# jdm365/Compression_Algorithms

Hardware: AMD Instinct MI355X
Metric: encode GB/s on enwik9 at 1/2/4/8 MI355X; ratio vs ref; round-trip bit-exact (higher is better)
Workload: dtype u8; 1 GPU; deflate (LZ77 W=32 KiB len<=31 + per-block dynamic Huffman over the 286-symbol alphabet, mode H), independent 64 KiB blocks; 1000000000 enwik-shaped bytes in the job, 1000000000 on rank 0; input_seed=12345, mode=H, input_bytes_job=1000000000, input_bytes_rank0=1000000000, compressed_bytes_job=516875560, compressed_bytes_rank0=516875560, gather_to_rank0=False, parallelism=blocks sharded over 1 GPU(s), weak scaling

## Files before the change

### compression_algorithms_amd/csrc/lz2.h

```cpp
#pragma once
#include "lz_common.h"

#define LZ2_NG_BITS   14
#define LZ2_NG        (1u << LZ2_NG_BITS)
#ifndef LZ2_CAP
#define LZ2_CAP       4096u
#endif
#ifndef LZ2_CAP_S
#define LZ2_CAP_S     2560u
#endif
#ifndef LZ2_THREADS
#define LZ2_THREADS   512
#endif
#define LZ2_NWAVES    (LZ2_THREADS / 64)
#ifndef LZ2_PARTBITS
#define LZ2_PARTBITS  7
#endif
#define LZ2_MAXPARTS  (1u << LZ2_PARTBITS)
static_assert(LZ2_CAP % LZ2_THREADS == 0 && LZ2_CAP_S % LZ2_THREADS == 0 && LZ2_CAP_S <= LZ2_CAP, "entries per thread must be whole");
static_assert(2u * (LZ_MAX_BLOCK / LZ2_CAP_S + 1u + 16u) + 2u <= LZ2_MAXPARTS, "a block could need more parts than the partition can number");
#define LZ2_GRID_PARTS 32u
#ifndef LZ2_BIG
#define LZ2_BIG       8u
#endif
#define LZ2_WAVE      128u
#define LZ2_MAXBIG    (LZ2_CAP / LZ2_BIG)
#define LZ2_BIG_STRIDE (2u * LZ_MAX_BLOCK)
#define LZ2_ALIGN8(x)  (((x) + 7u) & ~7u)
#define LZ2_DESC_SMALL (LZ_MAX_BLOCK / LZ2_BIG + 32u)
#define LZ2_NCLASS    8u
#define LZ2_BIG_SMALL 1024u
__host__ __device__ __forceinline__ uint32_t lz2_class_of(uint32_t cnt, uint32_t wave_min)
{
    const bool three = (wave_min >> 16) != 0u;
    wave_min &= 0xFFFFu;
    if (cnt >= wave_min) return cnt > LZ2_BIG_SMALL ? 6u : cnt >= 512u ? 4u : (three && cnt < 256u) ? 3u : 5u;
    return cnt < 16 ? 7u : cnt < 32 ? 0u : cnt < 64 ? 1u : cnt < 128 ? 2u : cnt < 256 ? 3u : 4u;
}

struct Lz2BlockMeta {
    uint32_t n, nparts, base, fallback;
    uint32_t nbig, nbig_entries;
    uint32_t pad[2];
    uint32_t part_start[LZ2_MAXPARTS];
    uint32_t part_count[LZ2_MAXPARTS];
    uint32_t part_lo[LZ2_MAXPARTS];
};

struct Lz2BigDesc {
    uint32_t block;
    uint32_t start;
    uint32_t count;
    uint32_t anom;
    uint32_t limit;
// ... 20 lines not shown
```

### compression_algorithms_amd/csrc/lz2_find.hip

```cpp
#include "lz_common.h"
#include "lz2.h"
#include "lz_dom.h"
#include "lz_replay.h"
#include <stdlib.h>

#define RS_HEAD 0x8000u
#define RS_MASK 0x7FFFu

__device__ __forceinline__ bool bm2_test(const uint32_t *bm, uint32_t b) { return (bm[b >> 5] >> (b & 31u)) & 1u; }

__device__ void replay_small(const uint16_t *pos, uint16_t *rs, const uint16_t *pid, uint16_t *occ, uint32_t *bm,
                             uint32_t s, uint32_t e, uint32_t W, uint32_t anom, uint32_t limit, uint16_t *cand_i)
{
    uint32_t ev = s;
    bool anom_pending = anom != ~0u;
    const bool plain = (anom == ~0u) && (limit == ~0u);
    if (plain && (uint32_t)pos[e - 1] <= (uint32_t)pos[s] + W) {
        for (uint32_t i = s; i < e; ++i) { const uint32_t id = pid[i]; cand_i[i] = (id != pos[i]) ? (uint16_t)id : (uint16_t)LZ_NONE16; }
        return;
    }
    for (uint32_t i = s; i < e; ++i) {
        const uint32_t p = pos[i], rsv = rs[i], r = rsv & RS_MASK, id = pid[i];
        while (ev < i && (uint32_t)pos[ev] + W < p) {
            const uint32_t b = rs[ev] & RS_MASK;
// ... 45 lines not shown
        const uint32_t i = s + li;
        const uint32_t p = pos[i], rr = ((uint32_t)rs[i] & RS_MASK) - s, id = pid[i];
        while (ev < li && ev_pos + W < p) {
            mask &= ~(1u << ((uint32_t)(slots >> (4u * ev)) & 15u));
            ++ev; ev_pos = pos[s + ev];
        }
        uint32_t res = LZ_NONE16;
        if (ev == 0) {
            if (id != p) res = id;
        } else if (id != p) {
            for (uint32_t b = rr; (mask >> b) & 1u; ++b) {
                const uint32_t o = s + ((uint32_t)(ent >> (4u * b)) & 15u);
                if (pid[o] == id) { res = pos[o]; break; }
            }
        }
        cand_i[i] = (uint16_t)res;
        const uint32_t b = rr + (uint32_t)__builtin_ctz(~(mask >> rr));
        mask |= 1u << b;
        ent = (ent & ~((F)15u << (4u * b))) | ((F)li << (4u * b));
        slots |= (F)b << (4u * li);
    }
}

template <uint32_t CAP>
__device__ __forceinline__ void lz2_find_part(const uint8_t *__restrict__ in, uint64_t n_total, const LzP &P, const Lz2Scratch &sc, uint64_t block0, const uint64_t item)
{
    __shared__ uint16_t s_pos[CAP];
    __shared__ uint32_t s_word[CAP];
    __shared__ uint16_t s_j0[CAP], s_j1[CAP];
    __shared__ __attribute__((aligned(16))) uint16_t s_gr[2 * CAP];
    uint16_t *const s_g = s_gr;
    uint16_t *const s_r = s_gr + CAP;
    __shared__ uint16_t s_pid[CAP + 2];
    __shared__ uint32_t s_cnt[LZ2_NWAVES + 1][256];
    __shared__ uint32_t s_bm[CAP / 32 + 2];
    __shared__ uint32_t s_mix[CAP / 32 + 2];
    __shared__ int32_t  s_i32[18];
    __shared__ uint32_t s_zslot, s_zgid, s_nbigl, s_ngroups;
    uint16_t *const s_gstart = s_pid;
    uint32_t *const s_big = &s_cnt[0][0];
    uint16_t *const s_quiet = reinterpret_cast<uint16_t *>(&s_cnt[0][0] + 3 * (CAP / LZ2_BIG));
    static_assert(3 * (CAP / LZ2_BIG) * 4 + 2 * (CAP / LZ2_BIG) * 2 <= sizeof(uint32_t) * LZ2_NWAVES * 256, "export lists must fit the radix counters");

    const int tid = threadIdx.x;
    const uint32_t lb = (uint32_t)item & 0xFFFFu, part = (uint32_t)(item >> 16) & 0xFFu;
    Lz2BlockMeta *mt = sc.meta + lb;
    long long tk = clock64();
#ifdef MI_MEASURE
#define LZ2_STOP(k) if ((k) < 7 && sc.stop_phase == (uint32_t)(k) + 1u) return
#else
#define LZ2_STOP(k) do { } while (0)
#endif
#define LZ2_TICK(k) do { if (sc.dbg && tid == 0) { long long t2 = clock64(); atomicAdd((unsigned long long *)&sc.dbg[k], (unsigned long long)(t2 - tk)); tk = t2; } \
                         LZ2_STOP(k); } while (0)
    const uint32_t m = (uint32_t)(item >> 24) & 0xFFFFu;
    if (m == 0) return;
    const uint32_t pstart = (uint32_t)(item >> 40), base = mt->base;
    const uint64_t off = (block0 + lb) * (uint64_t)P.block;
    const uint32_t nblk = mt->n;
    const uint8_t *src = in + off;
    const uint32_t T = 1u << P.tbits, Tmask = T - 1u, W = 1u << P.wbits;
    uint16_t *plist = sc.plist + (size_t)lb * LZ_MAX_BLOCK + pstart;
    (void)n_total;
    const uint32_t plo_ = mt->part_lo[part];
    const uint32_t phi_ = (part + 1 < mt->nparts) ? mt->part_lo[part + 1] : T;
    const bool three = (phi_ - plo_) > 65536u;
    uint32_t *const cntA = &s_cnt[0][0];
    uint32_t (*const s_cntB)[256] = reinterpret_cast<uint32_t (*)[256]>(s_gr);
    uint32_t *const cntB = &s_cntB[0][0];
    constexpr uint32_t RST = LZ2_NWAVES + 1;
    const uint32_t seg = radix_seg<LZ2_NWAVES>(m), seg_inv = (uint32_t)((0x100000000ull + seg - 1u) / seg);
    for (uint32_t i = tid; i < 256u * RST; i += LZ2_THREADS) { cntA[i] = 0; cntB[i] = 0; }

    bool viol = false;
    {
        constexpr uint32_t BPT = LZ_MAX_BLOCK / LZ2_THREADS;
        static_assert(BPT % 16u == 0, "whole 16-byte loads");
        const uint4 *pm = reinterpret_cast<const uint4 *>(sc.partmap + (size_t)lb * LZ_MAX_BLOCK + (size_t)tid * BPT);
        static_assert(BPT == 128u, "the match bitmap below is four dwords per thread");
        const uint32_t pat = part * 0x01010101u;
        auto nib = [&](uint32_t w) -> uint32_t {
            const uint32_t x = w ^ pat;
            const uint32_t z = ~(((x & 0x7F7F7F7Fu) + 0x7F7F7F7Fu) | x) & 0x80808080u;
            return (((z >> 7) * 0x00204081u) >> 21) & 15u;
        };
        uint32_t bm[4] = {0u, 0u, 0u, 0u};
        {
            uint4 pv[BPT / 16u];
#pragma unroll
            for (uint32_t q = 0; q < BPT / 16u; ++q) pv[q] = pm[q];
#pragma unroll
            for (uint32_t q = 0; q < BPT / 16u; ++q)
                bm[q >> 1] |= (nib(pv[q].x) | (nib(pv[q].y) << 4) | (nib(pv[q].z) << 8) | (nib(pv[q].w) << 12)) << (16u * (q & 1u));
        }
        const uint32_t mine = (uint32_t)(__popc(bm[0]) + __popc(bm[1]) + __popc(bm[2]) + __popc(bm[3]));
        __shared__ uint32_t s_scanp[LZ2_NWAVES + 2];
        uint32_t total_m;
        uint32_t at = block_exclusive_scan<uint32_t>(mine, OpAddU32(), 0u, s_scanp, &total_m);
        (void)total_m;
        const uint32_t p0 = (uint32_t)tid * BPT;
#pragma unroll
        for (uint32_t k = 0; k < 4; ++k) {
// ... 11 lines not shown
        constexpr uint32_t GCH = CAP / LZ2_THREADS;
        uint32_t gp[GCH], glo[GCH], ghi[GCH];
        const bool aligned = (((uintptr_t)src) & 3u) == 0;
#pragma unroll
        for (uint32_t c = 0; c < GCH; ++c) { const uint32_t j = tid + c * LZ2_THREADS; gp[c] = j < m ? (uint32_t)s_pos[j] : 0u; if (j < m) plist[j] = (uint16_t)gp[c]; }
#pragma unroll
        for (uint32_t c = 0; c < GCH; ++c) {
            const uint32_t j = tid + c * LZ2_THREADS, p = gp[c];
            glo[c] = 0; ghi[c] = 0;
            if (j < m) {
                if (p + 8 <= nblk && aligned) {
                    const uintptr_t a = (uintptr_t)(src + p) & ~(uintptr_t)3;
                    glo[c] = *reinterpret_cast<const uint32_t *>(a);
                    ghi[c] = *reinterpret_cast<const uint32_t *>(a + 4);
                } else {
                    uint32_t w = 0;
                    for (uint32_t k = 0; k < 4 && p + k < nblk; ++k) w |= (uint32_t)src[p + k] << (8 * k);
                    glo[c] = w;
                }
            }
        }
        __syncthreads();
#pragma unroll
        for (uint32_t c = 0; c < GCH; ++c) {
            const uint32_t j = tid + c * LZ2_THREADS, p = gp[c];
            if (j < m) {
                uint32_t w = glo[c];
                if (p + 8 <= nblk && aligned) {
                    const uint32_t sh = ((uint32_t)((uintptr_t)(src + p) & 3u)) * 8u;
                    if (sh) w = (glo[c] >> sh) | (ghi[c] << (32u - sh));
                }
                const uint32_t mx = lz_mix32(w);
                s_word[j] = mx;
                atomicAdd(&cntA[(((((mx & Tmask) - base) & Tmask) - plo_) & 255u) * RST + __umulhi(j, seg_inv)], 1u);
            }
        }
    }
    for (uint32_t i = tid; i < CAP / 32 + 2; i += LZ2_THREADS) { s_bm[i] = 0; s_mix[i] = 0; }
    if (tid == 0) { s_zslot = ~0u; s_zgid = ~0u; s_nbigl = 0; }
    __syncthreads();
    auto homep = [&](uint32_t j) -> uint32_t { return ((s_word[j] & Tmask) - base) & Tmask; };
    LZ2_TICK(0);

    const uint32_t arank = P.flags & (LZP_ARANK | LZP_BREAK);
    auto keyp = [&](uint32_t j) -> uint32_t { return homep(j) - plo_; };
    uint16_t *srt = s_j0;
    if (three) {
        radix_pass<LZ2_NWAVES, 8, uint32_t>(m, s_cnt, [&](uint32_t i) { return i; },
            [&](uint32_t e) { return keyp(e) & 255u; }, [&](uint32_t d, uint32_t e) { s_j0[d] = (uint16_t)e; }, arank, nullptr, true,
            [&](uint32_t d, uint32_t e) { atomicAdd(&cntB[((keyp(e) >> 8) & 255u) * RST + __umulhi(d, seg_inv)], 1u); });
        for (uint32_t i = tid; i < 256u * RST; i += LZ2_THREADS) cntA[i] = 0;
        radix_pass<LZ2_NWAVES, 8, uint32_t>(m, s_cntB, [&](uint32_t i) { return (uint32_t)s_j0[i]; },
            [&](uint32_t e) { return (keyp(e) >> 8) & 255u; }, [&](uint32_t d, uint32_t e) { s_j1[d] = (uint16_t)e; }, arank, nullptr, true,
            [&](uint32_t d, uint32_t e) { atomicAdd(&cntA[((keyp(e) >> 16) & 255u) * RST + __umulhi(d, seg_inv)], 1u); });
        radix_pass<LZ2_NWAVES, 8, uint32_t>(m, s_cnt, [&](uint32_t i) { return (uint32_t)s_j1[i]; },
            [&](uint32_t e) { return (keyp(e) >> 16) & 255u; }, [&](uint32_t d, uint32_t e) { s_j0[d] = (uint16_t)e; }, arank, nullptr, true);
    } else {
        radix_pass<LZ2_NWAVES, 8, uint32_t>(m, s_cnt, [&](uint32_t i) { return i; },
            [&](uint32_t e) { return keyp(e) & 255u; }, [&](uint32_t d, uint32_t e) { s_j1[d] = (uint16_t)e; }, arank, sc.dbg, true,
            [&](uint32_t d, uint32_t e) { atomicAdd(&cntB[((keyp(e) >> 8) & 255u) * RST + __umulhi(d, seg_inv)], 1u); });
        radix_pass<LZ2_NWAVES, 8, uint32_t>(m, s_cntB, [&](uint32_t i) { return (uint32_t)s_j1[i]; },
            [&](uint32_t e) { return (keyp(e) >> 8) & 255u; }, [&](uint32_t d, uint32_t e) { s_j0[d] = (uint16_t)e; }, arank, sc.dbg, true);
    }
    (void)srt;

    LZ2_TICK(1);
    constexpr uint32_t CH = CAP / LZ2_THREADS;
    const uint32_t k0 = tid * CH, k1 = (k0 + CH < m) ? k0 + CH : m;
    {
        uint32_t rj[CH], rw[CH]; int32_t rh[CH];
        int32_t mx = INT32_MIN;
#pragma unroll
        for (uint32_t c = 0; c < CH; ++c) {
            const uint32_t k = k0 + c;
            rj[c] = 0; rw[c] = 0; rh[c] = 0;
            if (k < k1) {
                rj[c] = s_j0[k]; rw[c] = s_word[rj[c]]; rh[c] = (int32_t)(((rw[c] & Tmask) - base) & Tmask);
                const int32_t g = rh[c] - (int32_t)k;
                mx = g > mx ? g : mx;
            }
        }
        int32_t gmax_total;
        const int32_t premax = block_exclusive_scan<int32_t>(mx, OpMaxI32(), INT32_MIN, s_i32, &gmax_total);
        int32_t prev_h0 = 0; uint32_t prev_j = 0;
        if (k0 > 0 && k0 < m) { prev_j = s_j0[k0 - 1]; prev_h0 = (int32_t)homep(prev_j); }
        uint32_t nheads = 0; int32_t lasthead = -1, lastrun = -1;
        {
            int32_t run = premax, prev_h = prev_h0;
#pragma unroll
            for (uint32_t c = 0; c < CH; ++c) {
                const uint32_t k = k0 + c;
                if (k < k1) {
                    const int32_t h = rh[c], g = h - (int32_t)k;
                    const bool head = (k == 0) || (g >= run);
                    run = g > run ? g : run;
// ... 57 lines not shown
                }
                s_pid[j] = s_pos[id];
            }
        }
    }
    if (viol) { lz_order_violation(P); viol = false; }
    __syncthreads();
    if (!P.deflate && W >= nblk) {
        uint16_t *cout = sc.cand + (size_t)lb * LZ_MAX_BLOCK + pstart;
        for (uint32_t j = tid; j < m; j += LZ2_THREADS) { const uint32_t id = s_pid[j]; cout[j] = (id != s_pos[j]) ? (uint16_t)id : (uint16_t)LZ_NONE16; }
        return;
    }
    if (tid == 0) {
        const uint32_t Z = (0u - base) & Tmask;
        const uint32_t plo = mt->part_lo[part];
        const uint32_t phi = (part + 1 < mt->nparts) ? mt->part_lo[part + 1] : T;
        if (Z >= plo && (Z < phi || phi == T)) {
            int32_t lo = -1, hi = (int32_t)m - 1;
            while (lo < hi) { const int32_t mid = (lo + hi + 1) >> 1; if (homep(s_j0[mid]) <= Z) lo = mid; else hi = mid - 1; }
            if (lo >= 0) {
                const uint32_t j = s_j0[lo], gid = s_g[j];
                const uint32_t slot = (uint32_t)s_r[j] + (Z - homep(j));
                int32_t a = lo, b = (int32_t)m - 1;
                while (a < b) { const int32_t mid = (a + b + 1) >> 1; if (s_g[s_j0[mid]] == gid) a = mid; else b = mid - 1; }
                if (slot <= (uint32_t)a) { s_zslot = slot; s_zgid = gid; }
            }
        }
    }
    __syncthreads();

    LZ2_TICK(2);
    static_assert(CAP <= 8192, "cluster numbers must fit 13 bits");
    constexpr int GB2 = CAP > 4096 ? 7 : 6;
    static_assert(2 * CAP <= sizeof(uint32_t) * (LZ2_NWAVES + 1) * 256, "the cluster cursors live in the radix counters");
    if (arank & LZP_ARANK) {
        uint32_t *cur32 = &s_cnt[0][0];
        const uint32_t wv = (uint32_t)tid >> 6, ln = (uint32_t)tid & 63u;
        auto multi = [&](uint32_t g) -> bool { return (s_bm[g >> 5] >> (g & 31u)) & 1u; };
        for (uint32_t k = k0; k < k1; ++k) { const uint32_t j = s_j0[k]; if (!multi(s_g[j])) s_j1[k] = (uint16_t)j; }
        __syncthreads();
        uint32_t nm;
        {
            uint32_t mine[CH], cnt = 0;
#pragma unroll
            for (uint32_t c = 0; c < CH; ++c) { const uint32_t j = k0 + c; mine[c] = (j < m && multi(s_g[j])) ? 1u : 0u; cnt += mine[c]; }
            uint32_t at = block_exclusive_scan<uint32_t>(cnt, OpAddU32(), 0u, reinterpret_cast<uint32_t *>(s_i32), &nm);
#pragma unroll
            for (uint32_t c = 0; c < CH; ++c) if (mine[c]) s_j0[at++] = (uint16_t)(k0 + c);
        }
        __syncthreads();
        for (uint32_t x0 = 0; x0 < nm; x0 += 256u) {
            uint32_t jj[4], gg[4], old[4];
#pragma unroll
            for (uint32_t u = 0; u < 4; ++u) { const uint32_t x = x0 + 64u * u + ln; jj[u] = x < nm ? (uint32_t)s_j0[x] : 0u; gg[u] = x < nm ? (uint32_t)s_g[jj[u]] : 0xFFFFFFFFu; }
#pragma unroll
            for (uint32_t u = 0; u < 4; ++u) {
                old[u] = 0;
                if (gg[u] != 0xFFFFFFFFu && ((gg[u] >> 1) % (uint32_t)LZ2_NWAVES) == wv) old[u] = atomicAdd(&cur32[gg[u] >> 1], 1u << (16u * (gg[u] & 1u)));
            }
#pragma unroll
            for (uint32_t u = 0; u < 4; ++u)
                if (gg[u] != 0xFFFFFFFFu && ((gg[u] >> 1) % (uint32_t)LZ2_NWAVES) == wv) s_j1[(old[u] >> (16u * (gg[u] & 1u))) & 0xFFFFu] = (uint16_t)jj[u];
        }
        __syncthreads();
        for (uint32_t i = tid; i < CAP / 32 + 2; i += LZ2_THREADS) s_bm[i] = 0;
    } else {
        radix_pass<LZ2_NWAVES, 6, uint32_t>(m, s_cnt, [&](uint32_t i) { return i; },
            [&](uint32_t e) { return (uint32_t)s_g[e] & 63u; }, [&](uint32_t d, uint32_t e) { s_j0[d] = (uint16_t)e; }, arank);
        radix_pass<LZ2_NWAVES, GB2, uint32_t>(m, s_cnt, [&](uint32_t i) { return (uint32_t)s_j0[i]; },
// ... 76 lines not shown
            for (int sz = (int)LZ2_BIG - 1; sz >= 2; --sz) { const uint32_t t = s_bin[sz]; s_bin[sz] = run; run += t; }
            s_ncl = run;
        }
        __syncthreads();
        for (uint32_t c = 0; c < CH; ++c)
            if (my_n[c] >= 2 && my_n[c] < LZ2_BIG) c_start[atomicAdd(&s_bin[my_n[c]], 1u)] = (uint16_t)my_s[c];
        __syncthreads();
        LZ2_TICK(12);
        nbig = s_nbigl < (CAP / LZ2_BIG) ? s_nbigl : (CAP / LZ2_BIG);
        {
            uint32_t it = 0;
            for (uint32_t q = tid; q < nbig; q += LZ2_THREADS, ++it) {
                const uint32_t cnt = s_big[3 * q + 1] - s_big[3 * q];
                const uint32_t cls = lz2_class_of(cnt, sc.wave_min);
                my_rank[it] = atomicAdd(&s_cls[cls], 1u);
                my_dst[it] = atomicAdd(&s_ent, LZ2_ALIGN8(cnt));
            }
        }
        __syncthreads();
        uint32_t pending_base = 0;
        const bool want_cls = tid < (int)LZ2_NCLASS && s_cls[tid], want_ent = tid == 32 && s_ent;
        if (want_cls || want_ent) {
            uint32_t *ap = want_ent ? &mt->nbig_entries : &sc.big_count[tid & (int)(LZ2_NCLASS - 1u)];
            pending_base = atomicAdd(ap, want_ent ? s_ent : s_cls[tid & (int)(LZ2_NCLASS - 1u)]);
        }
        if (want_ent) atomicAdd(&mt->nbig, nbig);
        for (uint32_t q = tid >> 6; q < s_nquiet; q += LZ2_NWAVES)
            for (uint32_t k = (uint32_t)s_quiet[2 * q] + (tid & 63u); k < s_quiet[2 * q + 1]; k += 64) {
                const uint32_t id = e_pid[k];
                cand_i[k] = (id != e_pos[k]) ? (uint16_t)id : (uint16_t)LZ_NONE16;
            }
        const uint32_t ncl = s_ncl;
        LZ2_TICK(13);
        if (sc.dbg && tid == 0) { atomicAdd((unsigned long long *)&sc.dbg[23], (unsigned long long)ncl); atomicAdd((unsigned long long *)&sc.dbg[24], (unsigned long long)nbig);
                                  atomicAdd((unsigned long long *)&sc.dbg[25], (unsigned long long)s_ent); atomicAdd((unsigned long long *)&sc.dbg[26], (unsigned long long)s_nquiet);
                                  atomicAdd((unsigned long long *)&sc.dbg[27], (unsigned long long)m); atomicAdd((unsigned long long *)&sc.dbg[28], (unsigned long long)s_ngroups); }
        for (uint32_t c = 0; c < CH; ++c) {
            const uint32_t i = tid + c * (uint32_t)LZ2_THREADS;
            if (i >= m) continue;
            const uint32_t g_ = regs[c][2] >> 16;
            if ((s_mix[g_ >> 5] >> (g_ & 31u)) & 1u) continue;
            const uint32_t s = s_gstart[g_];
            if (s == s_zhead || s_gstart[g_ + 1] - s < 2u) continue;
            const uint32_t p = regs[c][0];
            uint32_t a = e_pos[s], lo = s + 1u;
            while (a + W < p) {
                uint32_t hi = i;
                while (lo < hi) { const uint32_t mid = (lo + hi) >> 1; if ((uint32_t)e_pos[mid] > a + W) hi = mid; else lo = mid + 1u; }
                a = e_pos[lo]; ++lo;
            }
            cand_i[i] = (a == p) ? (uint16_t)LZ_NONE16 : (uint16_t)a;
        }
        for (uint32_t q = tid; q < ncl; q += LZ2_THREADS) {
            const uint32_t s = c_start[q];
            uint32_t e = s + 1;
            while (e < m && !(e_rs[e] & RS_HEAD)) ++e;
            const bool zc = (s == s_zhead);
            if (zc) replay_small(e_pos, e_rs, e_pid, occ, s_bm, s, e, W, s_zslot, P.deflate ? s_zslot : ~0u, cand_i);
            else if (LZ2_BIG > 8u && e - s >= 8u) replay_small_reg<uint64_t>(e_pos, e_rs, e_pid, s, e, W, cand_i);
            else replay_small_reg<uint32_t>(e_pos, e_rs, e_pid, s, e, W, cand_i);
        }
        if (want_cls) s_clsbase[tid] = pending_base;
        if (want_ent) s_entbase = pending_base;
    }
    __syncthreads();
    LZ2_TICK(5);
    {
        uint32_t it = 0;
        for (uint32_t q = tid; q < nbig; q += LZ2_THREADS, ++it) {
// ... 2 lines not shown
            const uint32_t dst = s_entbase + my_dst[it];
            s_big[3 * q + 2] = dst;
            Lz2BigDesc d;
            d.block = lb; d.start = dst; d.count = cnt;
            const bool zc = (s == s_zhead);
            d.anom = zc ? s_zslot - s : ~0u;
            d.limit = (zc && P.deflate) ? s_zslot - s : ~0u;
            d.pad[0] = pstart; d.pad[1] = d.pad[2] = 0;
            sc.desc[cls][s_clsbase[cls] + my_rank[it]] = d;
        }
    }
    __syncthreads();
    for (uint32_t b = tid >> 6; b < nbig; b += LZ2_NWAVES) {
        const uint32_t s = s_big[3 * b], e = s_big[3 * b + 1], dst = s_big[3 * b + 2];
        uint16_t *bp = sc.bigpos + (size_t)lb * LZ2_BIG_STRIDE + dst;
        uint16_t *br = sc.bigrs + (size_t)lb * LZ2_BIG_STRIDE + dst;
        uint16_t *bi = sc.bigpid + (size_t)lb * LZ2_BIG_STRIDE + dst;
        for (uint32_t i = s + (tid & 63); i < e; i += 64) {
            cand_i[i] = e_pos[i];
            bp[i - s] = e_pos[i];
            br[i - s] = (uint16_t)((e_rs[i] & RS_MASK) - s);
            bi[i - s] = e_pid[i];
        }
        uint16_t *bc = sc.bigcand + (size_t)lb * LZ2_BIG_STRIDE + dst;
        for (uint32_t k = (e - s) + (tid & 63); k < LZ2_ALIGN8(e - s); k += 64) { bp[k] = 0; bc[k] = 0; }
    }
    uint16_t *cand_j = s_pid;
    __syncthreads();
    for (uint32_t i = tid; i < m; i += LZ2_THREADS) cand_j[s_j1[i]] = cand_i[i];
    __syncthreads();
    uint16_t *cout = sc.cand + (size_t)lb * LZ_MAX_BLOCK + pstart;
    for (uint32_t j = tid; j < m; j += LZ2_THREADS) cout[j] = cand_j[j];
    LZ2_TICK(6);
    if (sc.dbg && tid == 0) atomicAdd((unsigned long long *)&sc.dbg[15], 1ull);
}


__global__ __launch_bounds__(LZ2_THREADS)
void k_lz2_find(const uint8_t *__restrict__ in, uint64_t n_total, LzP P, Lz2Scratch sc, uint64_t block0)
{
    const uint32_t listed = *sc.work_count, nwork = listed < gridDim.x ? listed : gridDim.x;
    const uint32_t cpx = (nwork + 7u) >> 3, item_idx = (blockIdx.x & 7u) * cpx + (blockIdx.x >> 3);
    if ((blockIdx.x >> 3) >= cpx || item_idx >= nwork) return;
    lz2_find_part<LZ2_CAP_S>(in, n_total, P, sc, block0, sc.work[item_idx]);
}

__global__ __launch_bounds__(LZ2_THREADS)
void k_lz2_find_wide(const uint8_t *__restrict__ in, uint64_t n_total, LzP P, Lz2Scratch sc, uint64_t block0, uint32_t covered)
{
    const uint32_t nwide = sc.work_count[1], listed = sc.work_count[0], rest = listed > covered ? listed - covered : 0u;
    for (uint32_t k = blockIdx.x; k < nwide + rest; k += gridDim.x) {
        lz2_find_part<LZ2_CAP>(in, n_total, P, sc, block0, k < nwide ? sc.work[sc.work_slots - 1u - k] : sc.work[covered + (k - nwide)]);
        __syncthreads();
    }
}

template <int LDS_ENTRIES, int NW>
__global__ __launch_bounds__(64)
void k_lz2_big(LzP P, Lz2Scratch sc, int large)
{
    __shared__ uint32_t s_occ[LDS_ENTRIES];
    __shared__ uint16_t s_slot[LDS_ENTRIES];
    const uint32_t lane = threadIdx.x;
    const uint32_t nhi = large == 1 ? sc.big_count[6] : (large == 2 || large == 4) ? 0u : sc.big_count[4],
                   ncl = nhi + ((large == 0 || large == 2) ? sc.big_count[5] : large == 4 ? sc.big_count[3] : 0u);
    const uint32_t W = 1u << P.wbits;
    for (uint32_t ci = blockIdx.x; ci < ncl; ci += gridDim.x) {
        const Lz2BigDesc *dp = large == 1 ? &sc.desc[6][ci] : large == 4 ? &sc.desc[3][ci] : (ci < nhi ? &sc.desc[4][ci] : &sc.desc[5][ci - nhi]);
        const uint32_t d_block = dp->block, d_start = dp->start, n = dp->count;
        if (n & 0x80000000u) continue;
        const uint32_t d_anom = dp->anom, d_limit = dp->limit;
// ... 458 lines not shown
```

### compression_algorithms_amd/csrc/lz_common.h

```cpp
#pragma once
#include "common.h"

#define LZ_MAX_BLOCK   65536u
#define LZ_TAIL        64u
#define LZ_NONE16      0xFFFFu

#define LZ_TILE_NOM    4096u
#define LZ_TILE_CAP    8192u
#define LZ_GIANT_MIN   (LZ_TILE_CAP - LZ_TILE_NOM)
#define LZ_GIANT_CAP   18432u
#define LZ_MAX_TILES   (LZ_MAX_BLOCK / LZ_TILE_NOM)
#define LZ_WAVE_MIN    128u
#define LZ_MAX_GIANTS_PER_BLOCK (LZ_MAX_BLOCK / LZ_WAVE_MIN + 32u)
#ifndef LZ_TILE_WAVE_MIN
#define LZ_TILE_WAVE_MIN 16u
#endif

struct LzP {
    uint32_t wbits, lbits, tbits, deflate, block;
    uint32_t flags;
    uint32_t *order_flag;
    uint64_t *stats;
};
#define LZP_ARANK 1u
#define LZP_BREAK 2u
#define LZP_FORCE_FB 4u

__device__ __forceinline__ void lz_order_violation(const LzP &P)
{
    if (P.order_flag) __hip_atomic_fetch_or(P.order_flag, 1u, __ATOMIC_RELAXED, __HIP_MEMORY_SCOPE_SYSTEM);
}

static inline LzP lz_params_of(mi_ctx *ctx, const mi_lz_params *p)
{
// ... 79 lines not shown

__device__ __forceinline__ void lz_block_to_lds(uint8_t *s_dst, const uint8_t *__restrict__ src, uint32_t n, uint32_t tid)
{
    constexpr uint32_t NIT = (LZ_MAX_BLOCK + LZ_TAIL + 1024u * 16u - 1u) / (1024u * 16u);
    const bool vec_ok = ((((uintptr_t)src) & 15u) == 0) && n >= 16u;
    if (vec_ok) {
        const uint32_t last = (n - 16u) & ~15u;
        uint4 v[NIT];
#pragma unroll
        for (uint32_t k = 0; k < NIT; ++k) {
            const uint32_t i = tid * 16u + k * 1024u * 16u;
            v[k] = *reinterpret_cast<const uint4 *>(src + (i <= last ? i : last));
        }
#pragma unroll
        for (uint32_t k = 0; k < NIT; ++k) {
            const uint32_t i = tid * 16u + k * 1024u * 16u;
            if (i >= LZ_MAX_BLOCK + LZ_TAIL) continue;
            if (i + 16u <= n) *reinterpret_cast<uint4 *>(s_dst + i) = v[k];
            else if (i >= n) *reinterpret_cast<uint4 *>(s_dst + i) = make_uint4(0u, 0u, 0u, 0u);
            else {
#pragma unroll 1
                for (uint32_t b = 0; b < 16; ++b) s_dst[i + b] = (i + b < n) ? src[i + b] : (uint8_t)0;
            }
        }
    } else {
#pragma unroll 1
        for (uint32_t i = tid * 16u; i < LZ_MAX_BLOCK + LZ_TAIL; i += 1024u * 16u) {
#pragma unroll 1
            for (uint32_t b = 0; b < 16; ++b) s_dst[i + b] = (i + b < n) ? src[i + b] : (uint8_t)0;
        }
    }
}

template <typename T, typename Op>
__device__ __forceinline__ T wave_inclusive_scan(T v, Op op)
{
    const int lane = threadIdx.x & 63;
#pragma unroll
    for (int o = 1; o < 64; o <<= 1) {
        T t = __shfl_up(v, o);
        if (lane >= o) v = op(t, v);
    }
    return v;
}

template <typename T, typename Op>
__device__ __forceinline__ T block_exclusive_scan(T v, Op op, T ident, T *s_tmp, T *total)
{
    const int lane = threadIdx.x & 63, wave = threadIdx.x >> 6, nw = (blockDim.x + 63) >> 6;
    T inc = wave_inclusive_scan(v, op);
    T exc = __shfl_up(inc, 1);
    if (lane == 0) exc = ident;
    if (lane == 63) s_tmp[wave] = inc;
    __syncthreads();
    if (threadIdx.x == 0) {
        T run = ident;
        for (int w = 0; w < nw; ++w) { T t = s_tmp[w]; s_tmp[w] = run; run = op(run, t); }
        s_tmp[nw] = run;
    }
    __syncthreads();
    T res = op(s_tmp[wave], exc);
    *total = s_tmp[nw];
    __syncthreads();
    return res;
}

struct OpAddU32 { __device__ uint32_t operator()(uint32_t a, uint32_t b) const { return a + b; } };
struct OpMaxI32 { __device__ int32_t operator()(int32_t a, int32_t b) const { return a > b ? a : b; } };

struct AffMax { int32_t a, b; };
__device__ __forceinline__ uint64_t am_pack(AffMax f) { return ((uint64_t)(uint32_t)f.a << 32) | (uint32_t)f.b; }
__device__ __forceinline__ AffMax am_unpack(uint64_t v) { AffMax f; f.a = (int32_t)(v >> 32); f.b = (int32_t)(uint32_t)v; return f; }
#define AM_NEG (-(1 << 28))
__device__ __forceinline__ AffMax am_then(AffMax first, AffMax second)
{
    AffMax r;
    r.a = first.a + second.a;
    if (r.a < AM_NEG) r.a = AM_NEG;
    int32_t t = first.b + second.a;
    if (t < AM_NEG) t = AM_NEG;
    r.b = t > second.b ? t : second.b;
    return r;
}
struct OpAm { __device__ uint64_t operator()(uint64_t earlier, uint64_t later) const { return am_pack(am_then(am_unpack(earlier), am_unpack(later))); } };

struct RadixNoHook { __device__ __forceinline__ void operator()(uint32_t, uint32_t) const {} };
template <int NWAVES> __device__ __forceinline__ uint32_t radix_seg(uint32_t n) { return ((n + (uint32_t)(NWAVES * 64) - 1u) / (uint32_t)(NWAVES * 64)) * 64u; }
template <int D, bool SKIP = false> struct RadixDepth { static constexpr int value = D; static constexpr bool skip_identity = SKIP; };
template <int NWAVES, int NBITS, typename E, typename CntRow, typename Load, typename Digit, typename Store, typename Hook = RadixNoHook, typename Depth = RadixDepth<1>>
__device__ __forceinline__ bool radix_pass(uint32_t n, CntRow *s_cnt, Load load, Digit digit, Store store, uint32_t arank = 0u , uint64_t *dbg = nullptr,
                                           bool counted = false, Hook hook = Hook(), Depth = Depth())
{
    long long tk_ = dbg ? clock64() : 0;
#define RP_TICK(k) do { if (dbg && threadIdx.x == 0) { long long t2 = clock64(); atomicAdd((unsigned long long *)&dbg[k], (unsigned long long)(t2 - tk_)); tk_ = t2; } } while (0)
    static_assert(sizeof(CntRow) / sizeof(uint32_t) >= (1u << NBITS), "counter row too narrow for the digit");
    constexpr int ND = 1 << NBITS;
    constexpr int NT = NWAVES * 64;
    constexpr int ST = NWAVES + 1;
    uint32_t *cnt = &s_cnt[0][0];
    const int tid = threadIdx.x, lane = tid & 63, wave = tid >> 6;
    const uint32_t seg = ((n + (uint32_t)NT - 1u) / (uint32_t)NT) * 64u;
    const uint32_t a = wave * seg, b = (a + seg < n) ? a + seg : n;
    if (!counted) {
        for (int i = tid; i < ND * ST; i += NT) cnt[i] = 0;
        __syncthreads();
        if constexpr (Depth::value > 1) {
            constexpr int D = Depth::value;
            for (uint32_t i = a + lane; i < b; i += 64u * D) {
                E ee[D]; uint32_t dg[D];
#pragma unroll
                for (int u = 0; u < D; ++u) ee[u] = load(i + 64u * u < b ? i + 64u * u : b - 1u);
#pragma unroll
                for (int u = 0; u < D; ++u) dg[u] = digit(ee[u]);
#pragma unroll
                for (int u = 0; u < D; ++u) {
                    const bool v = i + 64u * u < b;
                    const uint32_t d0 = (uint32_t)__builtin_amdgcn_readfirstlane((int)dg[u]);
                    const uint64_t live = __ballot(v);
                    if (__ballot(v && dg[u] != d0) == 0ull && (live & 1ull)) {
                        if (lane == 0) atomicAdd(&cnt[d0 * ST + wave], (uint32_t)__popcll(live));
                    } else if (v) atomicAdd(&cnt[dg[u] * ST + wave], 1u);
                }
            }
        } else
        for (uint32_t i = a + lane; i < b; i += 256) {
            uint32_t dg[4];
#pragma unroll
            for (int u = 0; u < 4; ++u) dg[u] = (i + 64u * u < b) ? digit(load(i + 64u * u)) : 0u;
#pragma unroll
            for (int u = 0; u < 4; ++u) if (i + 64u * u < b) atomicAdd(&cnt[dg[u] * ST + wave], 1u);
        }
    }
    __syncthreads();
    RP_TICK(8);
    uint32_t pre[NWAVES];
    uint32_t tot = 0;
    if (tid < ND) {
#pragma unroll
        for (int w = 0; w < NWAVES; ++w) pre[w] = cnt[tid * ST + w];
#pragma unroll
        for (int w = 0; w < NWAVES; ++w) { const uint32_t t = pre[w]; pre[w] = tot; tot += t; }
    }
    if constexpr (Depth::skip_identity) {
        if (__syncthreads_or((tid < ND && tot == n) ? 1 : 0)) return true;
    }
    __shared__ uint32_t s_scan[18];
    uint32_t total;
    const uint32_t base = block_exclusive_scan<uint32_t>(tid < ND ? tot : 0u, OpAddU32(), 0u, s_scan, &total);
    if (tid < ND) {
#pragma unroll
        for (int w = 0; w < NWAVES; ++w) cnt[tid * ST + w] = pre[w] + base;
    }
    __syncthreads();
    RP_TICK(9);
    if (arank & LZP_ARANK) {
        for (uint32_t i = a + lane; i < b; i += 256) {
            E ee[4]; uint32_t dg[4], sl[4];
#pragma unroll
            for (int u = 0; u < 4; ++u) { ee[u] = E{}; dg[u] = 0; if (i + 64u * u < b) { ee[u] = load(i + 64u * u); dg[u] = digit(ee[u]); } }
#pragma unroll
            for (int u = 0; u < 4; ++u) sl[u] = (i + 64u * u < b) ? atomicAdd(&cnt[dg[u] * ST + wave], 1u) : 0u;
#ifdef MI_TEST_HOOKS
            if (arank & LZP_BREAK) {
#pragma unroll
                for (int u = 0; u < 4; ++u) {
                    const bool v = i + 64u * u < b;
                    const uint32_t dn = __shfl_xor(dg[u], 1), sn = __shfl_xor(sl[u], 1);
                    const bool vn = __shfl_xor(v ? 1 : 0, 1) != 0;
                    if (v && vn && dn == dg[u]) sl[u] = sn;
                }
            }
#endif
#pragma unroll
            for (int u = 0; u < 4; ++u) if (i + 64u * u < b) { store(sl[u], ee[u]); hook(sl[u], (uint32_t)ee[u]); }
        }
        __syncthreads();
        RP_TICK(10);
        return false;
    }
    if constexpr (Depth::value > 1) {
        constexpr int D = Depth::value;
        for (uint32_t i0 = a; i0 < b; i0 += 64u * D) {
            E ee[D]; uint32_t dg[D];
#pragma unroll
            for (int u = 0; u < D; ++u) { const uint32_t i = i0 + 64u * u + lane; ee[u] = load(i < b ? i : b - 1u); }
#pragma unroll
            for (int u = 0; u < D; ++u) dg[u] = digit(ee[u]);
#pragma unroll
            for (int u = 0; u < D; ++u) {
                const bool valid = i0 + 64u * u + lane < b;
                const uint32_t d = dg[u];
                uint64_t mask = __ballot(valid);
                if (mask == 0ull) continue;
#pragma unroll
                for (int k = 0; k < NBITS; ++k) {
                    const bool bit = (d >> k) & 1u;
                    const uint64_t bal = __ballot(valid && bit);
                    mask &= bit ? bal : ~bal;
                }
                const uint64_t below = mask & ((1ull << lane) - 1ull);
                const uint32_t rank = __popcll(below), num = __popcll(mask);
                const int leader = __ffsll((unsigned long long)mask) - 1;
                uint32_t old = 0;
                if (valid && lane == leader) old = atomicAdd(&cnt[d * ST + wave], num);
                old = __shfl(old, leader < 0 ? 0 : leader);
                if (valid) { store(old + rank, ee[u]); hook(old + rank, (uint32_t)ee[u]); }
            }
        }
        __syncthreads();
        RP_TICK(10);
        return false;
    }
    E en{};
    uint32_t dn = 0;
    if (a + lane < b) { en = load(a + lane); dn = digit(en); }
    for (uint32_t i0 = a; i0 < b; i0 += 64) {
        const uint32_t i = i0 + lane;
        const bool valid = i < b;
        const E e = en;
        const uint32_t d = dn;
        if (i + 64 < b) { en = load(i + 64); dn = digit(en); }
        uint64_t mask = __ballot(valid);
#pragma unroll
        for (int k = 0; k < NBITS; ++k) {
            const bool bit = (d >> k) & 1u;
            const uint64_t bal = __ballot(valid && bit);
            mask &= bit ? bal : ~bal;
        }
        const uint64_t below = mask & ((1ull << lane) - 1ull);
        const uint32_t rank = __popcll(below), num = __popcll(mask);
        const int leader = __ffsll((unsigned long long)mask) - 1;
        uint32_t old = 0;
        if (valid && lane == leader) old = atomicAdd(&cnt[d * ST + wave], num);
        old = __shfl(old, leader < 0 ? 0 : leader);
        if (valid) { store(old + rank, e); hook(old + rank, (uint32_t)e); }
    }
    __syncthreads();
    RP_TICK(10);
    return false;
}


template <int NBITS, typename E, typename CntRow, typename Load, typename Digit, typename Store>
__device__ __forceinline__ void radix_pass_1024(uint32_t n, CntRow *s_cnt, Load load, Digit digit, Store store, uint32_t arank = 0u)
{
    (void)radix_pass<16, NBITS, E>(n, s_cnt, load, digit, store, arank, nullptr, false, RadixNoHook(), RadixDepth<4>());
}
template <int NBITS, typename E, typename CntRow, typename Load, typename Digit, typename Store>
__device__ __forceinline__ bool radix_pass_1024_or_skip(uint32_t n, CntRow *s_cnt, Load load, Digit digit, Store store)
{
    return radix_pass<16, NBITS, E>(n, s_cnt, load, digit, store, 0u, nullptr, false, RadixNoHook(), RadixDepth<4, true>());
}
```

Measured before the change: 22.04 GB/s.

## Shrink small-part LDS with 16-bit radix counters, DPP scans, more grid parts

Lowers the small-part capacity to 2048 entries and uses packed 16-bit radix counters for that instantiation, which shrinks shared memory per workgroup. Adds launch bounds so more workgroups fit per CU, and raises the grid part count to keep a full block covered. Replaces the shuffle-based wave scan with DPP row and broadcast operations and compiles debug timing hooks out of non-measure builds. The trade-offs are more parts per block (more launches of work items and more partition overhead) and packed-counter atomics that could overflow if counts ever exceed 16 bits.

```diff
diff --git a/compression_algorithms_amd/csrc/lz2.h b/compression_algorithms_amd/csrc/lz2.h
--- a/compression_algorithms_amd/csrc/lz2.h
+++ b/compression_algorithms_amd/csrc/lz2.h
@@ -7,7 +7,7 @@
 #define LZ2_CAP       4096u
 #endif
 #ifndef LZ2_CAP_S
-#define LZ2_CAP_S     2560u
+#define LZ2_CAP_S     2048u
 #endif
 #ifndef LZ2_THREADS
 #define LZ2_THREADS   512
@@ -19,7 +19,8 @@
 #define LZ2_MAXPARTS  (1u << LZ2_PARTBITS)
 static_assert(LZ2_CAP % LZ2_THREADS == 0 && LZ2_CAP_S % LZ2_THREADS == 0 && LZ2_CAP_S <= LZ2_CAP, "entries per thread must be whole");
 static_assert(2u * (LZ_MAX_BLOCK / LZ2_CAP_S + 1u + 16u) + 2u <= LZ2_MAXPARTS, "a block could need more parts than the partition can number");
-#define LZ2_GRID_PARTS 32u
+#define LZ2_GRID_PARTS 40u
+static_assert(LZ2_GRID_PARTS * LZ2_CAP_S >= 5u * LZ_MAX_BLOCK / 4u, "the grid must cover a full block of text with room to spare");
 #ifndef LZ2_BIG
 #define LZ2_BIG       8u
 #endif
diff --git a/compression_algorithms_amd/csrc/lz2_find.hip b/compression_algorithms_amd/csrc/lz2_find.hip
--- a/compression_algorithms_amd/csrc/lz2_find.hip
+++ b/compression_algorithms_amd/csrc/lz2_find.hip
@@ -101,15 +101,16 @@
     uint16_t *const s_g = s_gr;
     uint16_t *const s_r = s_gr + CAP;
     __shared__ uint16_t s_pid[CAP + 2];
-    __shared__ uint32_t s_cnt[LZ2_NWAVES + 1][256];
+    using Cnt = typename std::conditional<(CAP <= 2048u), uint16_t, uint32_t>::type;
+    __shared__ __attribute__((aligned(16))) Cnt s_cnt[LZ2_NWAVES + 1][256];
     __shared__ uint32_t s_bm[CAP / 32 + 2];
     __shared__ uint32_t s_mix[CAP / 32 + 2];
     __shared__ int32_t  s_i32[18];
     __shared__ uint32_t s_zslot, s_zgid, s_nbigl, s_ngroups;
     uint16_t *const s_gstart = s_pid;
-    uint32_t *const s_big = &s_cnt[0][0];
-    uint16_t *const s_quiet = reinterpret_cast<uint16_t *>(&s_cnt[0][0] + 3 * (CAP / LZ2_BIG));
-    static_assert(3 * (CAP / LZ2_BIG) * 4 + 2 * (CAP / LZ2_BIG) * 2 <= sizeof(uint32_t) * LZ2_NWAVES * 256, "export lists must fit the radix counters");
+    uint32_t *const s_big = reinterpret_cast<uint32_t *>(&s_cnt[0][0]);
+    uint16_t *const s_quiet = reinterpret_cast<uint16_t *>(s_big + 3 * (CAP / LZ2_BIG));
+    static_assert(3 * (CAP / LZ2_BIG) * 4 + 2 * (CAP / LZ2_BIG) * 2 <= sizeof(s_cnt), "export lists must fit the radix counters");
 
     const int tid = threadIdx.x;
     const uint32_t lb = (uint32_t)item & 0xFFFFu, part = (uint32_t)(item >> 16) & 0xFFu;
@@ -117,10 +118,12 @@
     long long tk = clock64();
 #ifdef MI_MEASURE
 #define LZ2_STOP(k) if ((k) < 7 && sc.stop_phase == (uint32_t)(k) + 1u) return
+#define LZ2_DBG     sc.dbg
 #else
 #define LZ2_STOP(k) do { } while (0)
+#define LZ2_DBG     ((uint64_t *)nullptr)
 #endif
-#define LZ2_TICK(k) do { if (sc.dbg && tid == 0) { long long t2 = clock64(); atomicAdd((unsigned long long *)&sc.dbg[k], (unsigned long long)(t2 - tk)); tk = t2; } \
+#define LZ2_TICK(k) do { if (LZ2_DBG && tid == 0) { long long t2 = clock64(); atomicAdd((unsigned long long *)&LZ2_DBG[k], (unsigned long long)(t2 - tk)); tk = t2; } \
                          LZ2_STOP(k); } while (0)
     const uint32_t m = (uint32_t)(item >> 24) & 0xFFFFu;
     if (m == 0) return;
@@ -134,9 +137,10 @@
     const uint32_t plo_ = mt->part_lo[part];
     const uint32_t phi_ = (part + 1 < mt->nparts) ? mt->part_lo[part + 1] : T;
     const bool three = (phi_ - plo_) > 65536u;
-    uint32_t *const cntA = &s_cnt[0][0];
-    uint32_t (*const s_cntB)[256] = reinterpret_cast<uint32_t (*)[256]>(s_gr);
-    uint32_t *const cntB = &s_cntB[0][0];
+    Cnt *const cntA = &s_cnt[0][0];
+    Cnt (*const s_cntB)[256] = reinterpret_cast<Cnt (*)[256]>(s_gr);
+    Cnt *const cntB = &s_cntB[0][0];
+    static_assert(sizeof(s_cnt) <= sizeof(s_gr), "the second pass's radix counters must fit s_g | s_r");
     constexpr uint32_t RST = LZ2_NWAVES + 1;
     const uint32_t seg = radix_seg<LZ2_NWAVES>(m), seg_inv = (uint32_t)((0x100000000ull + seg - 1u) / seg);
     for (uint32_t i = tid; i < 256u * RST; i += LZ2_THREADS) { cntA[i] = 0; cntB[i] = 0; }
@@ -214,7 +218,7 @@
                 }
                 const uint32_t mx = lz_mix32(w);
                 s_word[j] = mx;
-                atomicAdd(&cntA[(((((mx & Tmask) - base) & Tmask) - plo_) & 255u) * RST + __umulhi(j, seg_inv)], 1u);
+                radix_cnt_add(cntA, (((((mx & Tmask) - base) & Tmask) - plo_) & 255u) * RST + __umulhi(j, seg_inv), 1u);
             }
         }
     }
@@ -230,19 +234,19 @@
     if (three) {
         radix_pass<LZ2_NWAVES, 8, uint32_t>(m, s_cnt, [&](uint32_t i) { return i; },
             [&](uint32_t e) { return keyp(e) & 255u; }, [&](uint32_t d, uint32_t e) { s_j0[d] = (uint16_t)e; }, arank, nullptr, true,
-            [&](uint32_t d, uint32_t e) { atomicAdd(&cntB[((keyp(e) >> 8) & 255u) * RST + __umulhi(d, seg_inv)], 1u); });
+            [&](uint32_t d, uint32_t e) { radix_cnt_add(cntB, ((keyp(e) >> 8) & 255u) * RST + __umulhi(d, seg_inv), 1u); });
         for (uint32_t i = tid; i < 256u * RST; i += LZ2_THREADS) cntA[i] = 0;
         radix_pass<LZ2_NWAVES, 8, uint32_t>(m, s_cntB, [&](uint32_t i) { return (uint32_t)s_j0[i]; },
             [&](uint32_t e) { return (keyp(e) >> 8) & 255u; }, [&](uint32_t d, uint32_t e) { s_j1[d] = (uint16_t)e; }, arank, nullptr, true,
-            [&](uint32_t d, uint32_t e) { atomicAdd(&cntA[((keyp(e) >> 16) & 255u) * RST + __umulhi(d, seg_inv)], 1u); });
+            [&](uint32_t d, uint32_t e) { radix_cnt_add(cntA, ((keyp(e) >> 16) & 255u) * RST + __umulhi(d, seg_inv), 1u); });
         radix_pass<LZ2_NWAVES, 8, uint32_t>(m, s_cnt, [&](uint32_t i) { return (uint32_t)s_j1[i]; },
             [&](uint32_t e) { return (keyp(e) >> 16) & 255u; }, [&](uint32_t d, uint32_t e) { s_j0[d] = (uint16_t)e; }, arank, nullptr, true);
     } else {
         radix_pass<LZ2_NWAVES, 8, uint32_t>(m, s_cnt, [&](uint32_t i) { return i; },
-            [&](uint32_t e) { return keyp(e) & 255u; }, [&](uint32_t d, uint32_t e) { s_j1[d] = (uint16_t)e; }, arank, sc.dbg, true,
-            [&](uint32_t d, uint32_t e) { atomicAdd(&cntB[((keyp(e) >> 8) & 255u) * RST + __umulhi(d, seg_inv)], 1u); });
+            [&](uint32_t e) { return keyp(e) & 255u; }, [&](uint32_t d, uint32_t e) { s_j1[d] = (uint16_t)e; }, arank, LZ2_DBG, true,
+            [&](uint32_t d, uint32_t e) { radix_cnt_add(cntB, ((keyp(e) >> 8) & 255u) * RST + __umulhi(d, seg_inv), 1u); });
         radix_pass<LZ2_NWAVES, 8, uint32_t>(m, s_cntB, [&](uint32_t i) { return (uint32_t)s_j1[i]; },
-            [&](uint32_t e) { return (keyp(e) >> 8) & 255u; }, [&](uint32_t d, uint32_t e) { s_j0[d] = (uint16_t)e; }, arank, sc.dbg, true);
+            [&](uint32_t e) { return (keyp(e) >> 8) & 255u; }, [&](uint32_t d, uint32_t e) { s_j0[d] = (uint16_t)e; }, arank, LZ2_DBG, true);
     }
     (void)srt;
 
@@ -366,9 +370,9 @@
     LZ2_TICK(2);
     static_assert(CAP <= 8192, "cluster numbers must fit 13 bits");
     constexpr int GB2 = CAP > 4096 ? 7 : 6;
-    static_assert(2 * CAP <= sizeof(uint32_t) * (LZ2_NWAVES + 1) * 256, "the cluster cursors live in the radix counters");
+    static_assert(2 * CAP <= sizeof(s_cnt), "the cluster cursors live in the radix counters");
     if (arank & LZP_ARANK) {
-        uint32_t *cur32 = &s_cnt[0][0];
+        uint32_t *cur32 = reinterpret_cast<uint32_t *>(&s_cnt[0][0]);
         const uint32_t wv = (uint32_t)tid >> 6, ln = (uint32_t)tid & 63u;
         auto multi = [&](uint32_t g) -> bool { return (s_bm[g >> 5] >> (g & 31u)) & 1u; };
         for (uint32_t k = k0; k < k1; ++k) { const uint32_t j = s_j0[k]; if (!multi(s_g[j])) s_j1[k] = (uint16_t)j; }
@@ -511,9 +515,9 @@
             }
         const uint32_t ncl = s_ncl;
         LZ2_TICK(13);
-        if (sc.dbg && tid == 0) { atomicAdd((unsigned long long *)&sc.dbg[23], (unsigned long long)ncl); atomicAdd((unsigned long long *)&sc.dbg[24], (unsigned long long)nbig);
-                                  atomicAdd((unsigned long long *)&sc.dbg[25], (unsigned long long)s_ent); atomicAdd((unsigned long long *)&sc.dbg[26], (unsigned long long)s_nquiet);
-                                  atomicAdd((unsigned long long *)&sc.dbg[27], (unsigned long long)m); atomicAdd((unsigned long long *)&sc.dbg[28], (unsigned long long)s_ngroups); }
+        if (LZ2_DBG && tid == 0) { atomicAdd((unsigned long long *)&LZ2_DBG[23], (unsigned long long)ncl); atomicAdd((unsigned long long *)&LZ2_DBG[24], (unsigned long long)nbig);
+                                  atomicAdd((unsigned long long *)&LZ2_DBG[25], (unsigned long long)s_ent); atomicAdd((unsigned long long *)&LZ2_DBG[26], (unsigned long long)s_nquiet);
+                                  atomicAdd((unsigned long long *)&LZ2_DBG[27], (unsigned long long)m); atomicAdd((unsigned long long *)&LZ2_DBG[28], (unsigned long long)s_ngroups); }
         for (uint32_t c = 0; c < CH; ++c) {
             const uint32_t i = tid + c * (uint32_t)LZ2_THREADS;
             if (i >= m) continue;
@@ -582,11 +586,11 @@
     uint16_t *cout = sc.cand + (size_t)lb * LZ_MAX_BLOCK + pstart;
     for (uint32_t j = tid; j < m; j += LZ2_THREADS) cout[j] = cand_j[j];
     LZ2_TICK(6);
-    if (sc.dbg && tid == 0) atomicAdd((unsigned long long *)&sc.dbg[15], 1ull);
-}
-
-
-__global__ __launch_bounds__(LZ2_THREADS)
+    if (LZ2_DBG && tid == 0) atomicAdd((unsigned long long *)&LZ2_DBG[15], 1ull);
+}
+
+
+__global__ __launch_bounds__(LZ2_THREADS, 8)
 void k_lz2_find(const uint8_t *__restrict__ in, uint64_t n_total, LzP P, Lz2Scratch sc, uint64_t block0)
 {
     const uint32_t listed = *sc.work_count, nwork = listed < gridDim.x ? listed : gridDim.x;
diff --git a/compression_algorithms_amd/csrc/lz_common.h b/compression_algorithms_amd/csrc/lz_common.h
--- a/compression_algorithms_amd/csrc/lz_common.h
+++ b/compression_algorithms_amd/csrc/lz_common.h
@@ -1,5 +1,6 @@
 #pragma once
 #include "common.h"
+#include <type_traits>
 
 #define LZ_MAX_BLOCK   65536u
 #define LZ_TAIL        64u
@@ -145,15 +146,30 @@
     }
 }
 
+template <int CTRL, int ROW_MASK, typename T>
+__device__ __forceinline__ T dpp_move(T v, T old)
+{
+    static_assert(sizeof(T) % 4 == 0, "32-bit words");
+    uint32_t w[sizeof(T) / 4], o[sizeof(T) / 4];
+    __builtin_memcpy(w, &v, sizeof(T));
+    __builtin_memcpy(o, &old, sizeof(T));
+#pragma unroll
+    for (unsigned k = 0; k < sizeof(T) / 4; ++k)
+        w[k] = (uint32_t)__builtin_amdgcn_update_dpp((int)o[k], (int)w[k], CTRL, ROW_MASK, 0xF, false);
+    T r;
+    __builtin_memcpy(&r, w, sizeof(T));
+    return r;
+}
+
 template <typename T, typename Op>
-__device__ __forceinline__ T wave_inclusive_scan(T v, Op op)
-{
-    const int lane = threadIdx.x & 63;
-#pragma unroll
-    for (int o = 1; o < 64; o <<= 1) {
-        T t = __shfl_up(v, o);
-        if (lane >= o) v = op(t, v);
-    }
+__device__ __forceinline__ T wave_inclusive_scan(T v, Op op, T ident)
+{
+    v = op(dpp_move<0x111, 0xF>(v, ident), v);
+    v = op(dpp_move<0x112, 0xF>(v, ident), v);
+    v = op(dpp_move<0x114, 0xF>(v, ident), v);
+    v = op(dpp_move<0x118, 0xF>(v, ident), v);
+    v = op(dpp_move<0x142, 0xA>(v, ident), v);
+    v = op(dpp_move<0x143, 0xC>(v, ident), v);
     return v;
 }
 
@@ -161,9 +177,8 @@
 __device__ __forceinline__ T block_exclusive_scan(T v, Op op, T ident, T *s_tmp, T *total)
 {
     const int lane = threadIdx.x & 63, wave = threadIdx.x >> 6, nw = (blockDim.x + 63) >> 6;
-    T inc = wave_inclusive_scan(v, op);
-    T exc = __shfl_up(inc, 1);
-    if (lane == 0) exc = ident;
+    T inc = wave_inclusive_scan(v, op, ident);
+    T exc = dpp_move<0x138, 0xF>(inc, ident);
     if (lane == 63) s_tmp[wave] = inc;
     __syncthreads();
     if (threadIdx.x == 0) {
@@ -198,6 +213,12 @@
 struct OpAm { __device__ uint64_t operator()(uint64_t earlier, uint64_t later) const { return am_pack(am_then(am_unpack(earlier), am_unpack(later))); } };
 
 struct RadixNoHook { __device__ __forceinline__ void operator()(uint32_t, uint32_t) const {} };
+__device__ __forceinline__ uint32_t radix_cnt_add(uint32_t *cnt, uint32_t i, uint32_t v) { return atomicAdd(&cnt[i], v); }
+__device__ __forceinline__ uint32_t radix_cnt_add(uint16_t *cnt, uint32_t i, uint32_t v)
+{
+    const uint32_t sh = 16u * (i & 1u);
+    return (atomicAdd(reinterpret_cast<uint32_t *>(cnt) + (i >> 1), v << sh) >> sh) & 0xFFFFu;
+}
 template <int NWAVES> __device__ __forceinline__ uint32_t radix_seg(uint32_t n) { return ((n + (uint32_t)(NWAVES * 64) - 1u) / (uint32_t)(NWAVES * 64)) * 64u; }
 template <int D, bool SKIP = false> struct RadixDepth { static constexpr int value = D; static constexpr bool skip_identity = SKIP; };
 template <int NWAVES, int NBITS, typename E, typename CntRow, typename Load, typename Digit, typename Store, typename Hook = RadixNoHook, typename Depth = RadixDepth<1>>
@@ -206,11 +227,13 @@
 {
     long long tk_ = dbg ? clock64() : 0;
 #define RP_TICK(k) do { if (dbg && threadIdx.x == 0) { long long t2 = clock64(); atomicAdd((unsigned long long *)&dbg[k], (unsigned long long)(t2 - tk_)); tk_ = t2; } } while (0)
-    static_assert(sizeof(CntRow) / sizeof(uint32_t) >= (1u << NBITS), "counter row too narrow for the digit");
+    using C = std::remove_reference_t<decltype(s_cnt[0][0])>;
+    static_assert(std::is_same<C, uint32_t>::value || std::is_same<C, uint16_t>::value, "32- or 16-bit counters");
+    static_assert(sizeof(CntRow) / sizeof(C) >= (1u << NBITS), "counter row too narrow for the digit");
     constexpr int ND = 1 << NBITS;
     constexpr int NT = NWAVES * 64;
     constexpr int ST = NWAVES + 1;
-    uint32_t *cnt = &s_cnt[0][0];
+    C *cnt = &s_cnt[0][0];
     const int tid = threadIdx.x, lane = tid & 63, wave = tid >> 6;
     const uint32_t seg = ((n + (uint32_t)NT - 1u) / (uint32_t)NT) * 64u;
     const uint32_t a = wave * seg, b = (a + seg < n) ? a + seg : n;
@@ -231,8 +254,8 @@
                     const uint32_t d0 = (uint32_t)__builtin_amdgcn_readfirstlane((int)dg[u]);
                     const uint64_t live = __ballot(v);
                     if (__ballot(v && dg[u] != d0) == 0ull && (live & 1ull)) {
-                        if (lane == 0) atomicAdd(&cnt[d0 * ST + wave], (uint32_t)__popcll(live));
-                    } else if (v) atomicAdd(&cnt[dg[u] * ST + wave], 1u);
+                        if (lane == 0) radix_cnt_add(cnt, d0 * ST + wave, (uint32_t)__popcll(live));
+                    } else if (v) radix_cnt_add(cnt, dg[u] * ST + wave, 1u);
                 }
             }
         } else
@@ -241,7 +264,7 @@
 #pragma unroll
             for (int u = 0; u < 4; ++u) dg[u] = (i + 64u * u < b) ? digit(load(i + 64u * u)) : 0u;
 #pragma unroll
-            for (int u = 0; u < 4; ++u) if (i + 64u * u < b) atomicAdd(&cnt[dg[u] * ST + wave], 1u);
+            for (int u = 0; u < 4; ++u) if (i + 64u * u < b) radix_cnt_add(cnt, dg[u] * ST + wave, 1u);
         }
     }
     __syncthreads();
@@ -262,7 +285,7 @@
     const uint32_t base = block_exclusive_scan<uint32_t>(tid < ND ? tot : 0u, OpAddU32(), 0u, s_scan, &total);
     if (tid < ND) {
 #pragma unroll
-        for (int w = 0; w < NWAVES; ++w) cnt[tid * ST + w] = pre[w] + base;
+        for (int w = 0; w < NWAVES; ++w) cnt[tid * ST + w] = (C)(pre[w] + base);
     }
     __syncthreads();
     RP_TICK(9);
@@ -272,7 +295,7 @@
 #pragma unroll
             for (int u = 0; u < 4; ++u) { ee[u] = E{}; dg[u] = 0; if (i + 64u * u < b) { ee[u] = load(i + 64u * u); dg[u] = digit(ee[u]); } }
 #pragma unroll
-            for (int u = 0; u < 4; ++u) sl[u] = (i + 64u * u < b) ? atomicAdd(&cnt[dg[u] * ST + wave], 1u) : 0u;
+            for (int u = 0; u < 4; ++u) sl[u] = (i + 64u * u < b) ? radix_cnt_add(cnt, dg[u] * ST + wave, 1u) : 0u;
 #ifdef MI_TEST_HOOKS
             if (arank & LZP_BREAK) {
 #pragma unroll
@@ -315,7 +338,7 @@
                 const uint32_t rank = __popcll(below), num = __popcll(mask);
                 const int leader = __ffsll((unsigned long long)mask) - 1;
                 uint32_t old = 0;
-                if (valid && lane == leader) old = atomicAdd(&cnt[d * ST + wave], num);
+                if (valid && lane == leader) old = radix_cnt_add(cnt, d * ST + wave, num);
                 old = __shfl(old, leader < 0 ? 0 : leader);
                 if (valid) { store(old + rank, ee[u]); hook(old + rank, (uint32_t)ee[u]); }
             }
@@ -344,7 +367,7 @@
         const uint32_t rank = __popcll(below), num = __popcll(mask);
         const int leader = __ffsll((unsigned long long)mask) - 1;
         uint32_t old = 0;
-        if (valid && lane == leader) old = atomicAdd(&cnt[d * ST + wave], num);
+        if (valid && lane == leader) old = radix_cnt_add(cnt, d * ST + wave, num);
         old = __shfl(old, leader < 0 ? 0 : leader);
         if (valid) { store(old + rank, e); hook(old + rank, (uint32_t)e); }
     }
```

Result: faster. 23.13 GB/s, median of 6 (+4.9%).
